# Jiraiya812/Fast-CU-Decision-HEVC

Hardware: AMD Instinct MI355X
Metric: CTUs/sec (RDO decision only) at 4K all-intra (higher is better)
Workload: dtype int32+f64

## Files before the change

### fast-cu-decision-hevc_amd/csrc/fcu_engine.h

```cpp
#pragma once
#include <stdint.h>
#include <string.h>
#include <type_traits>
#include "../../include/fcu.h"

#ifdef FCU_EMU
#include <math.h>
#include <stdio.h>
#include <stdlib.h>
#define FCU_DEV static inline
#define FCU_MEMBER inline
#define FCU_NOINLINE
#define FCU_INLINE
#define FCU_TABLE static const
static int g_emu_phase = 0, g_emu_in_phase = 0, g_emu_lane = 0, g_emu_relax = 0;
#define FCU_EMU_RELAX(on) (g_emu_relax = (on))
static inline int fcu_emu_phase_begin() { g_emu_phase++; g_emu_in_phase = 1; g_emu_lane = 0; return 0; }
static inline int fcu_emu_phase_next(int lane) { if (lane + 1 >= 64) g_emu_in_phase = 0; g_emu_lane = lane + 1; return lane + 1; }
template <class T> static inline T fcu_emu_uni(T v, int site, int line)
{
  enum { SITES = 2048, K = 32, B = 16 };
  struct Seen { int phase, first, cur, idx, n; unsigned char vals[K][B]; };
  static Seen seen[SITES];
  if (g_emu_in_phase && !g_emu_relax && sizeof(T) <= B && site < SITES) {
// ... 927 lines not shown
        rdCodedLevelandDist += cc - cs;
        rdUncodedDist += c0;
        if (posInCG != 0) nnzBeforePos0++;
      }
    }
    if (lastScanPos >= 0 && cgScanPos > 0) {
      ctxSet = (uint32_t)((ch ? 4 : 0) + ((!ch && (cgScanPos - 1) > 0) ? 2 : 0) + (c1 == 0));
      c1 = 1; c2 = 0; c1Idx = 0; c2Idx = 0; goRice = 0;
    }
    if (cgLastScanPos >= 0) {
      if (cgScanPos) {
        if (((cgflag >> cgBlk) & 1) == 0) {
          const int ctxSig = cgBase + sig_cg_ctx(cgflag, cgx, cgy, wg);
          baseCost += lambda * (double)cb(ctxSig, 0) - rdSigCost;
          cgg[cgScanPos * st] = lambda * (double)cb(ctxSig, 0);
        } else if (cgScanPos < cgLastScanPos) {
          if (nnzBeforePos0 == 0) { baseCost -= rdSigCost0; rdSigCost -= rdSigCost0; }
          double costZeroCG = baseCost;
          const int ctxSig = cgBase + sig_cg_ctx(cgflag, cgx, cgy, wg);
          baseCost += lambda * (double)cb(ctxSig, 1);
          costZeroCG += lambda * (double)cb(ctxSig, 0);
          cgg[cgScanPos * st] = lambda * (double)cb(ctxSig, 1);
          costZeroCG += rdUncodedDist; costZeroCG -= rdCodedLevelandDist; costZeroCG -= rdSigCost;
          if (costZeroCG < baseCost) {
            cgflag &= ~(1ull << cgBlk); baseCost = costZeroCG;
            cgg[cgScanPos * st] = lambda * (double)cb(ctxSig, 0);
            for (int posInCG = 15; posInCG >= 0; posInCG--) {
              const int scanPos = cgScanPos * 16 + posInCG;
              if (SER) { if (g_S.rq_lv[posInCG]) { g_S.rq_lv[posInCG] = 0; g_S.rq_rec[posInCG].cc = g_S.rq_rec[posInCG].c0; g_S.rq_rec[posInCG].cs = 0; } }
              else if (dstg[scanPos * st]) { dstg[scanPos * st] = 0; recg[scanPos * st].cc = recg[scanPos * st].c0; recg[scanPos * st].cs = 0; }
            }
          }
        }
      } else cgflag |= 1ull << cgBlk;
    }
    if (SER) {
#pragma unroll
      for (int k = 0; k < 16; k++) { recg[(cgScanPos * 16 + k) * st] = g_S.rq_rec[k]; dstg[(cgScanPos * 16 + k) * st] = g_S.rq_lv[k]; }
    }
  }
  FCU_RTOC(P, rt_, 12);
  if (lastScanPos < 0) { RdoqOut z = { 0, -1 }; return z; }
  return rdoq_finish<SER>(cb, P, srcg, dstg, recg, cgg, st, log2, ch, scanType, cbfCtx, scan, scanCG, cgflag, cgLastScanPos, lastScanPos, baseCost, blockUncodedCost, lambda);
}

#ifdef FCU_EMU
template <class T> struct LaneVar {
  T v[64];
  LaneVar() { for (int i = 0; i < 64; i++) v[i] = T(); }
  void set(int lane, T x) { v[lane] = x; }
  T own(int lane) const { return v[lane]; }
  T get(int k) const { return v[k]; }
  void put(int k, T x) { v[k] = x; }
};
FCU_DEV uint32_t lane_mask16(const LaneVar<int> &f) { uint32_t m = 0; for (int k = 0; k < 16; k++) m |= (uint32_t)(f.v[k] != 0) << k; return m; }
#else
#if defined(__HIP_DEVICE_COMPILE__)
#define FCU_READLANE(v, k) __builtin_amdgcn_readlane((v), (k))
#define FCU_WRITELANE(val_, k_, old_) (((int)threadIdx.x == (k_)) ? (val_) : (old_))
#define FCU_BALLOT(p) __builtin_amdgcn_ballot_w64(p)
#else
#define FCU_READLANE(v, k) (v)
#define FCU_WRITELANE(val_, k_, old_) (val_)
#define FCU_BALLOT(p) ((unsigned long long)(p))
#endif
template <class T> struct LaneVar;
template <> struct LaneVar<int> {
  int r = 0;
  __device__ void set(int, int x) { r = x; }
  __device__ int own(int) const { return r; }
  __device__ int get(int k) const { return FCU_READLANE(r, k); }
  __device__ void put(int k, int x) { r = FCU_WRITELANE(x, k, r); }
};
template <> struct LaneVar<double> {
  double r = 0;
  __device__ void set(int, double x) { r = x; }
  __device__ double own(int) const { return r; }
  __device__ double get(int k) const
  { union { double d; int i[2]; } u; u.d = r; u.i[0] = FCU_READLANE(u.i[0], k); u.i[1] = FCU_READLANE(u.i[1], k); return u.d; }
  __device__ void put(int k, double x)
  { union { double d; int i[2]; } u, w; u.d = r; w.d = x; u.i[0] = FCU_WRITELANE(w.i[0], k, u.i[0]); u.i[1] = FCU_WRITELANE(w.i[1], k, u.i[1]); r = u.d; }
};
__device__ inline uint32_t lane_mask16(const LaneVar<int> &f) { return (uint32_t)FCU_BALLOT(f.r != 0) & 0xffffu; }
#endif

#ifndef FCU_WAVE_RDOQ_MIN_LOG2
#define FCU_WAVE_RDOQ_MIN_LOG2 2
#endif
FCU_DEV FCU_NOINLINE void rdoq_wave(int c, const int32_t *src, int16_t *dst, int topNZ, int log2, int comp, int scanType, int cbfCtx, const Params &P_, RdoqRec *rec, double *costCGSig)
{
  const Params &P = *FCU_UNI(&P_);
  c = FCU_UNI(c); src = FCU_UNI(src); dst = FCU_UNI(dst); topNZ = FCU_UNI(topNZ); log2 = FCU_UNI(log2); comp = FCU_UNI(comp);
  scanType = FCU_UNI(scanType); cbfCtx = FCU_UNI(cbfCtx); rec = FCU_UNI(rec); costCGSig = FCU_UNI(costCGSig);
  if (topNZ < 0) { FCU_SERIAL { g_S.rw_abs = 0; g_S.rw_lsp = -1; } return; }
  const FCU_HBM int32_t *srcg = (const FCU_HBM int32_t *)src; FCU_HBM int16_t *dstg = (FCU_HBM int16_t *)dst;
  FCU_HBM RdoqRec *recg = (FCU_HBM RdoqRec *)rec; FCU_HBM double *cgg = (FCU_HBM double *)costCGSig;
  auto cb = [&](int ctx, int bin) -> int { return (int)FCU_EST[ctx * 2 + bin]; };
  const int ch = comp ? 1 : 0, N = 1 << log2, n2 = N * N;
  const int qp = comp ? P.qp_c : P.qp;
  const int qbits = rdoq_qbits(log2, qp);
  const double lambda = P.rdoq_lambda[comp];
  const double errScale = P.err_scale[ch][log2 - 2];
  const uint16_t *scan = log2 == 2 ? &g_hot.scan[scanType][0] : k_scan + k_scan_off[scanType * 4 + log2 - 2];
  const uint8_t *scanCG = log2 <= 3 ? g_hot.scan_cg8[log2 == 2 ? 0 : scanType] : k_scan_cg + k_scan_cg_off[scanType * 4 + log2 - 2];
  const int wg = N >> 2, firstSig = first_sig_ctx(log2, scanType, ch);
  const int sigOff = CTX_SIG + (ch ? 28 : 0), cgBase = CTX_SIGCG + (ch ? 2 : 0);
  const uint64_t scan4 = g_hot.scan4_nib[scanType], map4 = g_hot.map4_nib;
  const int cgTop = topNZ >> 4;
  uint64_t cgflag = 0;
  int cgLastScanPos = -1; uint32_t ctxSet = 0; int c1 = 1, c2 = 0;
  double baseCost = 0, blockUncodedCost = 0;
  int lastScanPos = -1; uint32_t c1Idx = 0, c2Idx = 0, goRice = 0;
  int g10 = 0, g10Ctx = -1;
  for (int cg = (n2 >> 4) - 1; cg > cgTop; cg -= 4) {
    LaneVar<double> t0;
    FCU_FOR_LANES { const int g = cg - (lane >> 4); if (g > cgTop) { const double err = (double)iabs(srcg[g * 16 + (lane & 15)]); t0.set(lane, err * err * errScale); } }
    for (int j = 0; j < 4 && cg - j > cgTop; j++)
      for (int k = 15; k >= 0; k--) blockUncodedCost += t0.get(j * 16 + k);
  }
  baseCost = blockUncodedCost;
  LaneVar<int> vCgBlk, vNext;
  LaneVar<double> vCgSig;
  FCU_FOR_LANES { if (lane <= cgTop) vCgBlk.set(lane, scanCG[lane]); if (lane < 16) vNext.set(lane, srcg[cgTop * 16 + lane]); }
  for (int cgScanPos = cgTop; cgScanPos >= 0; cgScanPos--) {
    const int cgBlk = vCgBlk.get(cgScanPos), cgy = cgBlk / wg, cgx = cgBlk - cgy * wg;
    const int sigBase = sigOff + firstSig + ((!ch && (cgx + cgy) > 0) ? 3 : 0);
    const uint32_t cntBits = g_hot.cnt_bits[pattern_sig_ctx(cgflag, cgx, cgy, wg)];
    LaneVar<int> vLd, vMax, vSb0, vSb1, vUp, vDn, vSd, vDu, vLv, vCand;
    LaneVar<double> vC0, vCs, vCc;
    FCU_FOR_LANES {
      if (lane < 16) {
        const int posInCG = lane, scanPos = cgScanPos * 16 + posInCG;
        const int32_t levelDouble = iabs(vNext.own(lane));
        if (cgScanPos > 0) vNext.set(lane, srcg[scanPos - 16]);
        uint32_t maxAbsLevel = (uint32_t)((levelDouble + ((int32_t)1 << (qbits - 1))) >> qbits);
        if (maxAbsLevel > 32767u) maxAbsLevel = 32767u;
// ... 139 lines not shown
        if (lane <= top) {
          const int scanPos = cgScanPos * 16 + lane;
          const int lv = dstg[scanPos];
          const RdoqRec q = recg[scanPos];
          wLv.set(lane, lv); wCs.set(lane, q.cs); wCc.set(lane, q.cc); wC0.set(lane, q.c0);
          double costLast = 0;
          if (lv) {
            const int blk = scan[scanPos];
            const int py = blk >> log2, px = blk - (py << log2);
            const int ax = scanType == 2 ? py : px, ay = scanType == 2 ? px : py;
            const int gx = g_hot.group_idx[ax], gy = g_hot.group_idx[ay];
            int bxs = 0, bys = 0;
            for (int k = 0; k < gx; k++) bxs += cb(lbx + (k >> lsh), 1);
            if (gx < lgmax) bxs += cb(lbx + (gx >> lsh), 0);
            for (int k = 0; k < gy; k++) bys += cb(lby + (k >> lsh), 1);
            if (gy < lgmax) bys += cb(lby + (gy >> lsh), 0);
            double r = (double)(bxs + bys);
            if (gx > 3) r += 32768.0 * (double)((gx - 2) >> 1);
            if (gy > 3) r += 32768.0 * (double)((gy - 2) >> 1);
            costLast = lambda * r;
          }
          wCl.set(lane, costLast);
        }
      }
      for (int posInCG = top; posInCG >= 0; posInCG--) {
        const int lv = wLv.get(posInCG); const double curCs = wCs.get(posInCG);
        if (lv) {
          const double totalCost = baseCost + wCl.get(posInCG) - curCs;
          if (totalCost < bestCost) { bestLastIdxP1 = cgScanPos * 16 + posInCG + 1; bestCost = totalCost; }
          if (lv > 1) { foundLast = 1; break; }
          baseCost -= wCc.get(posInCG); baseCost += wC0.get(posInCG);
        } else baseCost -= curCs;
      }
    }
  }
  FCU_SERIAL { g_S.rw_abs = 0; }
  FCU_FOR_LANES {
    uint32_t acc = 0;
    for (int sp = lane; sp <= lastScanPos; sp += 64) {
      if (sp < bestLastIdxP1) { const int lv = dstg[sp]; acc += (uint32_t)lv; dstg[sp] = (int16_t)((srcg[sp] < 0) ? -lv : lv); }
      else dstg[sp] = 0;
    }
    FCU_WAVE_ADD((uint32_t *)&g_S.rw_abs, acc);
  }
  FCU_SERIAL {
    const int absSum = g_S.rw_abs;
    rdoq_sign_hiding(P, srcg, dstg, recg, 1, ch, bestLastIdxP1, absSum);
    int last = bestLastIdxP1 - 1;
    while (last >= 0 && dstg[last] == 0) last--;
    g_S.rw_lsp = last;
  }
}

FCU_DEV int use_filtered_ref(int mode, int log2, int isLuma)
{
  if (!isLuma || mode == DC) return 0;
  const int d1 = iabs(mode - HOR), d2 = iabs(mode - VER);
  return (d1 < d2 ? d1 : d2) > k_filter_thr[log2 - 2];
}
FCU_DEV int pred_pixel(const uint8_t *ref, int log2, int mode, int isLuma, int dc, int x, int y)
{
  const int N = 1 << log2;
  const uint8_t *corner = ref + 2 * N;
  if (mode == PLANAR)
    return ((N - 1 - x) * corner[-1 - y] + (x + 1) * corner[1 + N] + (N - 1 - y) * corner[1 + x] + (y + 1) * corner[-1 - N] + N) >> (log2 + 1);
  if (mode == DC) {
    int v = dc;
    if (isLuma && N <= 16) {
      if (x == 0 && y == 0) v = (corner[1] + corner[-1] + 2 * dc + 2) >> 2;
      else if (y == 0) v = (corner[1 + x] + 3 * dc + 2) >> 2;
      else if (x == 0) v = (corner[-1 - y] + 3 * dc + 2) >> 2;
    }
    return v;
  }
  const int isVer = mode >= 18;
  const int angMode = isVer ? mode - VER : -(mode - HOR);
  const int absAng = iabs(angMode);
  const int angAbs = (int)((0x2069544d245080ull >> (6 * absAng)) & 63);
  const int invAngle = absAng == 0 ? 0 : (int)(((absAng <= 4 ? 0x13b0e38ccd000ull : 0x8004ec30c1e2ull) >> (13 * ((absAng - 1) & 3))) & 8191);
  const int angle = angMode < 0 ? -angAbs : angAbs;
  const int px = isVer ? x : y, py = isVer ? y : x, ms = isVer ? 1 : -1;
  if (angle == 0) {
    int v = corner[ms * (px + 1)];
    if (isLuma && N <= 16 && px == 0) v = clip8(v + ((corner[-ms * (py + 1)] - corner[0]) >> 1));
    return v;
  }
  const int deltaPos = (py + 1) * angle, di = deltaPos >> 5, df = deltaPos & 31;
  const int i0 = px + di + 1;
  int r0, r1;
  { int i = i0; r0 = (i >= 0) ? corner[ms * i] : corner[-ms * ((128 + (-i) * invAngle) >> 8)]; }
  if (!df) return r0;
  { int i = i0 + 1; r1 = (i >= 0) ? corner[ms * i] : corner[-ms * ((128 + (-i) * invAngle) >> 8)]; }
  return ((32 - df) * r0 + df * r1 + 16) >> 5;
}

FCU_DEV int unit_available(const Env E, int lx, int ly, int cx, int cy)
{
  const Params &P = E.C->p;
  if (lx < 0 || ly < 0 || lx >= P.width || ly >= P.height) return 0;
  const int ctuN = (ly >> 6) * E.C->w_ctu + (lx >> 6), ctuC = (cy >> 6) * E.C->w_ctu + (cx >> 6);
  if (ctuN < E.slice_start) return 0;
  if (ctuN < ctuC) return 1;
  if (ctuN > ctuC) return 0;
  return zidx_of(lx, ly) < zidx_of(cx, cy);
}

// ... 778 lines not shown
      while (shift < numFull && cost < candCost[numFull - 1 - shift]) shift++;
      if (shift != 0) {
        for (int i = 1; i < shift; i++) { g_S.rd_mode[numFull - i] = g_S.rd_mode[numFull - 1 - i]; candCost[numFull - i] = candCost[numFull - 1 - i]; }
        g_S.rd_mode[numFull - shift] = mode; candCost[numFull - shift] = cost;
      }
    }
    for (int j = 0; j < nm; j++) {
      int inc = 0;
      for (int i = 0; i < numFull; i++) inc |= (preds[j] == g_S.rd_mode[i]);
      if (!inc) g_S.rd_mode[numFull++] = preds[j];
    }
    g_S.n_rd = numFull;
  }
}

FCU_DEV FCU_NOINLINE void pu_first_pass_batched(CuObj *cu, uint32_t tu_k)
{
  const Env E = env_get(); cu = FCU_UNI(cu); const TU tu = tu_of_key(FCU_UNI(tu_k));
  Scratch *G = E.G; const Params &P = E.C->p;
  const int d = cu->depth_cu, N = 1 << tu.log2, log2 = tu.log2, n2 = N * N, part = tu.part;
  const int partSize = cu->part_size[part];
  int checkTS = P.transform_skip && log2 == 2;
  if (P.ts_fast) checkTS = checkTS && (partSize == SIZE_NxN);
  const int nc = g_S.n_rd, tsv = checkTS ? 2 : 1, tss = tsv - 1, nvc = nc * tsv;
  FCU_CHECK(nvc <= MAXVC && nvc * n2 <= POOL && (MAXLC % 2) == 0);
  const int qbits = rdoq_qbits(log2, P.qp), qscale = k_quant_scales[P.qp % 6];
  const int useDst = log2 == 2;
  const uint8_t *org = G->org[d].y + tu.y * 64 + tu.x;
  build_ref(0, cu->x + tu.x, cu->y + tu.y, log2, 1);
  FCU_FOR_LANES {
    const int dc = g_S.dc;
    for (int i = lane; i < nc * n2; i += 64) {
      const int cnd = i / n2, p = i - cnd * n2, y = p >> log2, x = p & (N - 1), mode = g_S.rd_mode[cnd];
      const uint8_t *r = use_filtered_ref(mode, log2, 1) ? g_S.reff : g_S.ref;
      const int v = pred_pixel(r, log2, mode, 1, dc, x, y);
      G->p_pred[i] = (uint8_t)v; G->p_resi[i] = (int16_t)(org[y * 64 + x] - v);
    }
  }
  FCU_FOR_LANES { if (lane < nvc) g_S.vc_last[lane] = -1; by_log2(log2, [&](auto L) { constexpr int LG = decltype(L)::value; RowCache<(1 << LG), int16_t> rc; for (int i = lane; i < nc * n2; i += 64) { const int cnd = i / n2; G->p_tmp[i] = fwd1<LG>(rc, G->p_resi + cnd * n2, useDst, i - cnd * n2); } }); }
  FCU_FOR_LANES {
    est_build(CAB_CUR0 + d, lane);
    by_log2(log2, [&](auto L) { constexpr int LG = decltype(L)::value; RowCache<(1 << LG), int32_t> rc;
      for (int i = lane; i < nvc * n2; i += 64) {
        const int v = i / n2, p = i - v * n2, cnd = (v >> tss), ts = (v & tss);
        const uint16_t *iscan = k_iscan + k_scan_off[coef_scan_idx(g_S.rd_mode[cnd], log2, 0) * 4 + log2 - 2];
        const int32_t t = ts ? ((int32_t)G->p_resi[cnd * n2 + p] << (15 - 8 - log2)) : fwd2<LG>(rc, G->p_tmp + cnd * n2, useDst, p);
        const int sp = iscan[p]; const int32_t ld = level_double(t, qscale, qbits);
        G->p_lscan[sp * nvc + v] = ld;
        if (level_nonzero(ld, qbits)) FCU_ATOMIC_MAX(&g_S.vc_last[v], sp);
      }
    });
  }
  FCU_TIC(t2_);
  FCU_FOR_LANES {
    if (lane < nvc) {
      const int mode = g_S.rd_mode[(lane >> tss)];
      RdoqRec *rrec = G->r_rec + lane; double *rcg = G->r_cg + lane;
      const int cbfCtx = CTX_CBF_LUMA + (tu.tr_depth == 0 ? 1 : 0);
      const RdoqOut o = ((lane & tss) ? P.rdoq_ts : P.rdoq) ? rdoq<0, 1>(CAB_CUR0 + d, G->p_lscan + lane, G->p_qscan + lane, nvc, g_S.vc_last[lane], log2, 0, coef_scan_idx(mode, log2, 0), cbfCtx, P, rrec, rcg)
                                                            : quant_plain(G->p_lscan + lane, G->p_qscan + lane, nvc, g_S.vc_last[lane], log2, 0, P);
      g_S.vc_abs[lane] = o.abs_sum; g_S.vc_lsp[lane] = o.last;
      g_S.vc_dist[lane] = 0;
    }
    if (lane == 0) E.C->n_tu_trials += (unsigned long long)nvc;
  }
  FCU_TOC(E, t2_, 2);
  FCU_FOR_LANES {
    const DeqParams dq = deq_params(log2, P.qp);
    for (int i = lane; i < nvc * n2; i += 64) {
      const int v = i / n2, p = i - v * n2;
      const uint16_t *iscan = k_iscan + k_scan_off[coef_scan_idx(g_S.rd_mode[(v >> tss)], log2, 0) * 4 + log2 - 2];
      const int sp = iscan[p];
      const int q = (g_S.vc_abs[v] > 0 && (sp >> 4) <= (g_S.vc_last[v] >> 4)) ? G->p_qscan[sp * nvc + v] : 0;
      G->p_tmp[((v & tss)) ? i : v * n2 + tr_index(p, log2)] = dequant1(q, dq);
    }
  }
  FCU_FOR_LANES {
    by_log2(log2, [&](auto L) { constexpr int LG = decltype(L)::value; RowCache<(1 << LG), int32_t> rc;
      for (int i = lane; i < nvc * n2; i += 64) {
        const int v = i / n2, p = i - v * n2, ts = (v & tss);
        if (ts) { const int s = 15 - 8 - log2; G->p_tcoef[i] = (G->p_tmp[i] + (1 << (s - 1))) >> s; }
        else G->p_tcoef[i] = inv1<LG>(rc, G->p_tmp + v * n2, useDst, p);
      }
    });
  }
  FCU_FOR_LANES {
    by_log2(log2, [&](auto L) {
      uint32_t acc = 0;
      for (int i = lane; i < nvc * n2; i += 64) {
        const int v = i / n2, p = i - v * n2, cnd = (v >> tss), ts = (v & tss), y = p >> log2, x = p & (N - 1);
        int res = 0;
        if (g_S.vc_abs[v] > 0) res = ts ? (int16_t)G->p_tcoef[i] : inv2<decltype(L)::value>(G->p_tcoef + v * n2, useDst, p);
        const int r = clip8(G->p_pred[cnd * n2 + p] + res);
        G->p_rec[i] = (uint8_t)r;
        const int e = org[y * 64 + x] - r;
        FCU_DIST_ADD(acc, v, e, i, n2);
      }
    });
  }
  FCU_TIC(t3_);
  for (int vbase = 0; vbase < nvc; vbase += MAXLC) {
    const int slotBase = vbase ? (g_S.vc_slot[g_S.pu_best_vc] + 1) % MAXLC : 0;
#if defined(FCU_EMU) && defined(FCU_EMU_TRACE_ROUNDS)
    if (vbase) fprintf(stderr, "second bit-count round: %d variants\n", nvc);
#endif
    FCU_FOR_LANES {
      const int vc = vbase + lane;
      if (lane < MAXLC && vc < nvc) {
        const int cnd = (vc >> tss), ts = (vc & tss), mode = g_S.rd_mode[cnd], cbf = g_S.vc_abs[vc] > 0;
        const int slot = (slotBase + lane) % MAXLC;
        double cost;
        g_S.vc_slot[vc] = (uint8_t)slot;
        if (ts && !cbf) cost = FCU_MAX_DOUBLE;
        else {
          const int c = CAB_LANE0 + slot;
          cab_copy1(&g_S.cab[c], slot_ptr(E, d, CI_CURR_BEST));
          cab_reset_bits(c);
          if (part == 0 && P.slice_type != SLICE_I) { code_skip_flag(E, c, cu, 0); code_pred_mode(c, cu, 0); }
// ... 31 lines not shown
      }
      for (int i = lane; i < tu.nparts; i += 64) { G->tmp_tr_idx[i] = (uint8_t)tu.tr_depth; G->tmp_cbf[i] = (uint8_t)(cbf << tu.tr_depth); G->tmp_tskip[i] = (uint8_t)ts; }
    }
  }
}

FCU_DEV FCU_NOINLINE void pu_first_pass_64(CuObj *cu, uint32_t root_k)
{
  const Env E = env_get(); cu = FCU_UNI(cu); const TU root = tu_of_key(FCU_UNI(root_k));
  Scratch *G = E.G; const Params &P = E.C->p;
  const int d = cu->depth_cu, nc = g_S.n_rd, log2 = 5, N = 32, n2 = N * N, partSize = cu->part_size[root.part];
  FCU_CHECK(nc <= 5 && nc * n2 <= POOL && root.log2 == 6);
  const int qbits = rdoq_qbits(log2, P.qp), qscale = k_quant_scales[P.qp % 6];
  uint8_t *recpic = E.C->rec[0] + cu->y * E.C->stride[0] + cu->x; const int rs = E.C->stride[0];
  FCU_FOR_LANES {
    if (lane < nc) { const int c = CAB_LANE0 + lane; cab_copy1(&g_S.cab[c], slot_ptr(E, d, CI_CURR_BEST)); cab_reset_bits(c); g_S.c64_dist[lane] = 0; }
  }
  for (int k = 0; k < 4; k++) {
    TU tu; tu_child(tu, root, k, 0);
    const uint8_t *org = G->org[d].y + tu.y * 64 + tu.x;
    for (int cand = 0; cand < nc; cand++) {
      const int mode = g_S.rd_mode[cand], filt = use_filtered_ref(mode, log2, 1);
      if (k) {
        FCU_FOR_LANES {
          for (int i = lane; i < k * n2; i += 64) {
            const int j = i >> 10, q = i & (n2 - 1), yy = (j >> 1) * N + (q >> log2), xx = (j & 1) * N + (q & (N - 1));
            recpic[yy * rs + xx] = G->c64_rec[cand][yy * 64 + xx];
          }
        }
      }
      build_ref(0, cu->x + tu.x, cu->y + tu.y, log2, filt);
      FCU_FOR_LANES {
        const uint8_t *r = filt ? g_S.reff : g_S.ref; const int dc = g_S.dc;
        for (int i = lane; i < n2; i += 64) {
          const int y = i >> log2, x = i & (N - 1);
          const int v = pred_pixel(r, log2, mode, 1, dc, x, y);
          G->p_pred[cand * n2 + i] = (uint8_t)v; G->p_resi[cand * n2 + i] = (int16_t)(org[y * 64 + x] - v);
        }
      }
    }
    FCU_FOR_LANES { if (lane < nc) g_S.vc_last[lane] = -1; by_log2(log2, [&](auto L) { constexpr int LG = decltype(L)::value; RowCache<(1 << LG), int16_t> rc; for (int i = lane; i < nc * n2; i += 64) { const int cnd = i / n2; G->p_tmp[i] = fwd1<LG>(rc, G->p_resi + cnd * n2, 0, i - cnd * n2); } }); }
    FCU_FOR_LANES {
      by_log2(log2, [&](auto L) { constexpr int LG = decltype(L)::value; RowCache<(1 << LG), int32_t> rc;
        for (int i = lane; i < nc * n2; i += 64) {
          const int v = i / n2, p = i - v * n2;
          const uint16_t *iscan = k_iscan + k_scan_off[coef_scan_idx(g_S.rd_mode[v], log2, 0) * 4 + log2 - 2];
          const int32_t t = fwd2<LG>(rc, G->p_tmp + v * n2, 0, p);
          const int sp = iscan[p]; const int32_t ld = level_double(t, qscale, qbits);
          G->p_lscan[sp * nc + v] = ld;
          if (level_nonzero(ld, qbits)) FCU_ATOMIC_MAX(&g_S.vc_last[v], sp);
        }
      });
    }
    FCU_FOR_LANES {
      if (lane < nc) {
        RdoqRec *rrec = G->r_rec + lane; double *rcg = G->r_cg + lane;
        const RdoqOut o = P.rdoq ? rdoq<0, 0>(CAB_LANE0 + lane, G->p_lscan + lane, G->p_qscan + lane, nc, g_S.vc_last[lane], log2, 0,
                                              coef_scan_idx(g_S.rd_mode[lane], log2, 0), CTX_CBF_LUMA + (tu.tr_depth == 0 ? 1 : 0), P, rrec, rcg)
                                 : quant_plain(G->p_lscan + lane, G->p_qscan + lane, nc, g_S.vc_last[lane], log2, 0, P);
        g_S.vc_abs[lane] = o.abs_sum; g_S.vc_lsp[lane] = o.last; g_S.vc_dist[lane] = 0;
      }
      if (lane == 0) E.C->n_tu_trials += (unsigned long long)nc;
    }
    FCU_FOR_LANES {
      const DeqParams dq = deq_params(log2, P.qp);
      for (int i = lane; i < nc * n2; i += 64) {
        const int v = i / n2, p = i - v * n2;
        const uint16_t *iscan = k_iscan + k_scan_off[coef_scan_idx(g_S.rd_mode[v], log2, 0) * 4 + log2 - 2];
        const int sp = iscan[p];
        const int q = (g_S.vc_abs[v] > 0 && (sp >> 4) <= (g_S.vc_last[v] >> 4)) ? G->p_qscan[sp * nc + v] : 0;
        G->c64_coef[v][tu.off_y + sp] = (int16_t)q;
        G->p_tmp[v * n2 + tr_index(p, log2)] = dequant1(q, dq);
      }
    }
    FCU_FOR_LANES { by_log2(log2, [&](auto L) { constexpr int LG = decltype(L)::value; RowCache<(1 << LG), int32_t> rc; for (int i = lane; i < nc * n2; i += 64) { const int v = i / n2; G->p_tcoef[i] = inv1<LG>(rc, G->p_tmp + v * n2, 0, i - v * n2); } }); }
    FCU_FOR_LANES {
      by_log2(log2, [&](auto L) {
        uint32_t acc = 0;
        for (int i = lane; i < nc * n2; i += 64) {
          const int v = i / n2, p = i - v * n2, y = p >> log2, x = p & (N - 1);
          const int res = g_S.vc_abs[v] > 0 ? inv2<decltype(L)::value>(G->p_tcoef + v * n2, 0, p) : 0;
          const int r = clip8(G->p_pred[i] + res);
          G->c64_rec[v][(tu.y + y) * 64 + tu.x + x] = (uint8_t)r;
          const int e = org[y * 64 + x] - r;
          FCU_DIST_ADD(acc, v, e, i, n2);
        }
      });
    }
    FCU_FOR_LANES {
      if (lane < nc) {
        const int c = CAB_LANE0 + lane, mode = g_S.rd_mode[lane], cbf = g_S.vc_abs[lane] > 0;
        if (tu.part == 0 && P.slice_type != SLICE_I) { code_skip_flag(E, c, cu, 0); code_pred_mode(c, cu, 0); }
        if (tu.part == 0 && d == MAXDEPTH) cab_bin(c, partSize == SIZE_2Nx2N, CTX_PARTSIZE);
        if (tu.part == 0) code_luma_dir_bits(c, mode, g_S.preds);
        if (log2 != LOG2_MINTU && log2 != min_tu_log2_in_cu(d, partSize)) cab_bin(c, 0, CTX_SUBDIV + 5 - log2);
        cab_bin(c, cbf, CTX_CBF_LUMA + (tu.tr_depth == 0 ? 1 : 0));
        if (cbf) code_coeff_nxn<0>(c, G->p_qscan + lane, nc, g_S.vc_lsp[lane], log2, 0, coef_scan_idx(mode, log2, 0), 0, P, g_S.lane_abs[lane]);
        g_S.c64_dist[lane] += g_S.vc_dist[lane]; g_S.c64_cbf[lane][k] = (uint8_t)cbf;
        G->c64_distk[lane][k] = g_S.vc_dist[lane]; cab_copy1(&G->c64_state[lane][k], &g_S.cab[c]);
      }
    }
  }
  FCU_SERIAL {
    double best = FCU_MAX_DOUBLE; int bv = 0;
    for (int cand = 0; cand < nc; cand++) {
      const double c = rd_cost(P, (uint32_t)(g_S.cab[CAB_LANE0 + cand].frac >> 15), g_S.c64_dist[cand]);
      if (c < best) { best = c; bv = cand; }
    }
    g_S.pu_best_vc = bv; g_S.pu_best_cost = best; g_S.pu_best_dist = g_S.c64_dist[bv]; g_S.pu_best_mode = g_S.rd_mode[bv];
    g_S.c64_valid = 1;
  }
  {
    const int bv = g_S.pu_best_vc;
    Yuv *reco = &G->reco[d][1 - g_S.reco_best_idx[d]];
    const int any = g_S.c64_cbf[bv][0] | g_S.c64_cbf[bv][1] | g_S.c64_cbf[bv][2] | g_S.c64_cbf[bv][3];
    FCU_FOR_LANES {
// ... 152 lines not shown
    }
  }
  FCU_EMU_RELAX(0);
  return cab_bits(c);
}

FCU_DEV FCU_NOINLINE void chroma_leaf_trials(CuObj *cu, uint32_t tu_k)
{
  const Env E = env_get(); cu = FCU_UNI(cu); const TU tu = tu_of_key(FCU_UNI(tu_k));
  Scratch *G = E.G; const Params &P = E.C->p;
  const int d = cu->depth_cu;
  const int N = tu.cw, log2 = ilog2(N), n2 = N * N, trDepth = tu.tr_depth;
  int checkTS = P.transform_skip && N <= 4;
  if (P.ts_fast) {
    checkTS = checkTS && (tu.log2 == 2);
    if (checkTS) { int nb = 0; const int maxp = tu.part + (tu.c_code_all ? 1 : 4); for (int p = tu.part; p < maxp; p++) nb += cu->tskip[0][p]; checkTS = checkTS && (nb > 0); }
  }
  const int tsv = checkTS ? 2 : 1, tss = tsv - 1;
  const int perRound = (tsv == 1 && 10 * n2 <= POOL) ? 2 : 1;
  const int nm = 5 * perRound, nvc = nm * tsv;
  const int qbits = rdoq_qbits(log2, P.qp_c), qscale = k_quant_scales[P.qp_c % 6];
  const int subPart = tu_part_c(tu), nPartsC = tu_nparts_c(tu);
  const int lumaDir = cu->intra_dir[0][tu.part & ~3];
  for (int comp0 = 1; comp0 < 3; comp0 += perRound) {
    const int px = (cu->x >> 1) + tu.cx, py = (cu->y >> 1) + tu.cy;
    for (int cc = 0; cc < perRound; cc++) {
      const int comp = comp0 + cc;
      const uint8_t *org = yuv_plane(&G->org[d], comp) + tu.cy * 32 + tu.cx;
      chroma_leaf_refs5(E, cu, comp, px, py, log2);
      FCU_FOR_LANES {
        for (int i = lane; i < 5 * n2; i += 64) {
          const int m = i / n2, p = i - m * n2, y = p >> log2, x = p & (N - 1);
          const int mode = g_S.c_modes[m] == DM_CHROMA ? lumaDir : g_S.c_modes[m];
          const int pr = pred_pixel(g_S.ref5[m], log2, mode, 0, g_S.dc5[m], x, y);
          G->p_pred[cc * 5 * n2 + i] = (uint8_t)pr; G->p_resi[cc * 5 * n2 + i] = (int16_t)(org[y * 32 + x] - pr);
        }
      }
    }
    FCU_FOR_LANES { if (lane < nvc) g_S.vc_last[lane] = -1; by_log2(log2, [&](auto L) { constexpr int LG = decltype(L)::value; RowCache<(1 << LG), int16_t> rc; for (int i = lane; i < nm * n2; i += 64) { const int b = i / n2; G->p_tmp[i] = fwd1<LG>(rc, G->p_resi + b * n2, 0, i - b * n2); } }); }
    FCU_FOR_LANES {
      by_log2(log2, [&](auto L) { constexpr int LG = decltype(L)::value; RowCache<(1 << LG), int32_t> rc;
        for (int i = lane; i < nvc * n2; i += 64) {
          const int v = i / n2, p = i - v * n2, b = (v >> tss), ts = (v & tss), m = b % 5, comp = comp0 + b / 5;
          const int mode = g_S.c_modes[m] == DM_CHROMA ? lumaDir : g_S.c_modes[m];
          const uint16_t *iscan = k_iscan + k_scan_off[coef_scan_idx(mode, log2, comp) * 4 + log2 - 2];
          const int32_t t = ts ? ((int32_t)G->p_resi[b * n2 + p] << (15 - 8 - log2)) : fwd2<LG>(rc, G->p_tmp + b * n2, 0, p);
          const int sp = iscan[p]; const int32_t ld = level_double(t, qscale, qbits);
          G->p_lscan[sp * nvc + v] = ld;
          if (level_nonzero(ld, qbits)) FCU_ATOMIC_MAX(&g_S.vc_last[v], sp);
        }
      });
    }
    FCU_TIC(t13_);
    FCU_FOR_LANES {
      if (lane < nvc) {
        const int b = (lane >> tss), m = b % 5, comp = comp0 + b / 5;
        const int mode = g_S.c_modes[m] == DM_CHROMA ? lumaDir : g_S.c_modes[m];
        RdoqRec *rrec = G->r_rec + lane; double *rcg = G->r_cg + lane;
        const RdoqOut o = ((lane & tss) ? P.rdoq_ts : P.rdoq)
          ? rdoq<0, 0>(CAB_LANE0 + m, G->p_lscan + lane, G->p_qscan + lane, nvc, g_S.vc_last[lane], log2, 1 , coef_scan_idx(mode, log2, comp), CTX_CBF_CHROMA + trDepth, P, rrec, rcg)
          : quant_plain(G->p_lscan + lane, G->p_qscan + lane, nvc, g_S.vc_last[lane], log2, 1, P);
        g_S.vc_abs[lane] = o.abs_sum; g_S.vc_lsp[lane] = o.last;
        g_S.vc_dist[lane] = 0;
      }
      if (lane == 0) E.C->n_tu_trials += (unsigned long long)nvc;
    }
    FCU_TOC(E, t13_, 13);
    FCU_FOR_LANES {
      const DeqParams dq = deq_params(log2, P.qp_c);
      for (int i = lane; i < nvc * n2; i += 64) {
        const int v = i / n2, p = i - v * n2, b = (v >> tss), m = b % 5, comp = comp0 + b / 5;
        const int mode = g_S.c_modes[m] == DM_CHROMA ? lumaDir : g_S.c_modes[m];
        const uint16_t *iscan = k_iscan + k_scan_off[coef_scan_idx(mode, log2, comp) * 4 + log2 - 2];
        const int sp = iscan[p];
        const int q = (g_S.vc_abs[v] > 0 && (sp >> 4) <= (g_S.vc_last[v] >> 4)) ? G->p_qscan[sp * nvc + v] : 0;
        G->p_tmp[((v & tss)) ? i : v * n2 + tr_index(p, log2)] = dequant1(q, dq);
      }
    }
    FCU_FOR_LANES {
      by_log2(log2, [&](auto L) { constexpr int LG = decltype(L)::value; RowCache<(1 << LG), int32_t> rc;
        for (int i = lane; i < nvc * n2; i += 64) {
          const int v = i / n2, p = i - v * n2, ts = (v & tss);
          if (ts) { const int sft = 15 - 8 - log2; G->p_tcoef[i] = (G->p_tmp[i] + (1 << (sft - 1))) >> sft; }
          else G->p_tcoef[i] = inv1<LG>(rc, G->p_tmp + v * n2, 0, p);
        }
      });
    }
    FCU_FOR_LANES {
      by_log2(log2, [&](auto L) {
        uint32_t acc = 0;
        for (int i = lane; i < nvc * n2; i += 64) {
          const int v = i / n2, p = i - v * n2, b = (v >> tss), ts = (v & tss), y = p >> log2, x = p & (N - 1);
          const uint8_t *org = yuv_plane(&G->org[d], comp0 + b / 5) + tu.cy * 32 + tu.cx;
          int res = 0;
          if (g_S.vc_abs[v] > 0) res = ts ? (int16_t)G->p_tcoef[i] : inv2<decltype(L)::value>(G->p_tcoef + v * n2, 0, p);
          const int r = clip8(G->p_pred[b * n2 + p] + res);
          G->p_rec[i] = (uint8_t)r;
          const int e = org[y * 32 + x] - r;
          FCU_DIST_ADD(acc, v, e, i, n2);
        }
      });
    }
    FCU_FOR_LANES {
      if (lane < 5) {
        const int m = lane; int bestTs = 0;
        const int mode = g_S.c_modes[m] == DM_CHROMA ? lumaDir : g_S.c_modes[m];
        if (tsv == 2) {
          const int comp = comp0;
          uint32_t dsel = (uint32_t)(P.chroma_weight * (double)g_S.vc_dist[m * 2]);
          const uint32_t d0 = dsel, d1 = (uint32_t)(P.chroma_weight * (double)g_S.vc_dist[m * 2 + 1]);
          const int c0 = CAB_LANE0 + 5 + m, c1 = CAB_LANE0 + 10 + m;
          cab_copy1(&g_S.cab[c0], &g_S.cab[CAB_LANE0 + m]); cab_reset_bits(c0);
          if (g_S.vc_abs[m * 2] > 0) code_coeff_nxn<0>(c0, G->p_qscan + m * 2, nvc, g_S.vc_lsp[m * 2], log2, comp, coef_scan_idx(mode, log2, comp), 0, P, g_S.lane_abs[lane]);
          const double cost0 = rd_cost(P, cab_bits(c0), d0);
          double cost1 = FCU_MAX_DOUBLE;
          if (g_S.vc_abs[m * 2 + 1] > 0) {
            cab_copy1(&g_S.cab[c1], &g_S.cab[CAB_LANE0 + m]); cab_reset_bits(c1);
            code_coeff_nxn<0>(c1, G->p_qscan + m * 2 + 1, nvc, g_S.vc_lsp[m * 2 + 1], log2, comp, coef_scan_idx(mode, log2, comp), 1, P, g_S.lane_abs[lane]);
            cost1 = rd_cost(P, cab_bits(c1), d1);
// ... 517 lines not shown
```

Baseline: 18580.

## Batch RDOQ across candidates with lane-parallel sig-context precompute

Replaces the per-lane serial RDOQ call for each candidate TU with a batched walker. All candidates advance coefficient group by coefficient group in lockstep. Within each group, spare wave lanes precompute level magnitudes and significance bit costs for several scan positions at once. They also write records for zero coefficients directly, and the owning lanes then consume these values through ds_bpermute. The aim is to cut serial per-lane latency and divergence when nvc is much smaller than the wave width, at the cost of more lane shuffles, extra per-lane state and a large new code path.

```diff
diff --git a/fast-cu-decision-hevc_amd/csrc/fcu_engine.h b/fast-cu-decision-hevc_amd/csrc/fcu_engine.h
--- a/fast-cu-decision-hevc_amd/csrc/fcu_engine.h
+++ b/fast-cu-decision-hevc_amd/csrc/fcu_engine.h
@@ -1003,17 +1003,21 @@
   T own(int lane) const { return v[lane]; }
   T get(int k) const { return v[k]; }
   void put(int k, T x) { v[k] = x; }
+  T pull(int k) const { return v[k]; }
 };
 FCU_DEV uint32_t lane_mask16(const LaneVar<int> &f) { uint32_t m = 0; for (int k = 0; k < 16; k++) m |= (uint32_t)(f.v[k] != 0) << k; return m; }
+template <class T> struct LaneOwn { T v[64]; T &at(int lane) { return v[lane]; } };
 #else
 #if defined(__HIP_DEVICE_COMPILE__)
 #define FCU_READLANE(v, k) __builtin_amdgcn_readlane((v), (k))
 #define FCU_WRITELANE(val_, k_, old_) (((int)threadIdx.x == (k_)) ? (val_) : (old_))
 #define FCU_BALLOT(p) __builtin_amdgcn_ballot_w64(p)
+#define FCU_PULL(v, k) __builtin_amdgcn_ds_bpermute((k) << 2, (v))
 #else
 #define FCU_READLANE(v, k) (v)
 #define FCU_WRITELANE(val_, k_, old_) (val_)
 #define FCU_BALLOT(p) ((unsigned long long)(p))
+#define FCU_PULL(v, k) (v)
 #endif
 template <class T> struct LaneVar;
 template <> struct LaneVar<int> {
@@ -1022,6 +1026,7 @@
   __device__ int own(int) const { return r; }
   __device__ int get(int k) const { return FCU_READLANE(r, k); }
   __device__ void put(int k, int x) { r = FCU_WRITELANE(x, k, r); }
+  __device__ int pull(int k) const { return FCU_PULL(r, k); }
 };
 template <> struct LaneVar<double> {
   double r = 0;
@@ -1033,6 +1038,7 @@
   { union { double d; int i[2]; } u, w; u.d = r; w.d = x; u.i[0] = FCU_WRITELANE(w.i[0], k, u.i[0]); u.i[1] = FCU_WRITELANE(w.i[1], k, u.i[1]); r = u.d; }
 };
 __device__ inline uint32_t lane_mask16(const LaneVar<int> &f) { return (uint32_t)FCU_BALLOT(f.r != 0) & 0xffffu; }
+template <class T> struct LaneOwn { T r; __device__ T &at(int) { return r; } };
 #endif
 
 #ifndef FCU_WAVE_RDOQ_MIN_LOG2
@@ -1278,6 +1284,238 @@
   }
 }
 
+FCU_DEV int rdoq_batch_desc(int coder, int scanType, int useRdoq) { return coder | (scanType << 8) | (useRdoq << 10); }
+struct RdoqWalk {
+  uint64_t cgflag;
+  double baseCost, blockUncodedCost, rdSigCost, rdSigCost0, rdCodedLevelandDist, rdUncodedDist;
+  int cgTop, cgBlk, cgLastScanPos, lastScanPos, c1, c2, g10, g10Ctx, nnzBeforePos0, nzMask;
+  uint32_t ctxSet, c1Idx, c2Idx, goRice;
+};
+template <int EST>
+FCU_DEV FCU_NOINLINE void rdoq_batch(LaneVar<int> vDesc, int nvc, int log2, int comp, int cbfCtx, const Params &P_, const int32_t *src, int16_t *dst, RdoqRec *rec, double *costCGSig)
+{
+  const Params &P = *FCU_UNI(&P_);
+  nvc = FCU_UNI(nvc); log2 = FCU_UNI(log2); comp = FCU_UNI(comp); cbfCtx = FCU_UNI(cbfCtx);
+  src = FCU_UNI(src); dst = FCU_UNI(dst); rec = FCU_UNI(rec); costCGSig = FCU_UNI(costCGSig);
+  const FCU_HBM int32_t *srcg = (const FCU_HBM int32_t *)src; FCU_HBM int16_t *dstg = (FCU_HBM int16_t *)dst;
+  FCU_HBM RdoqRec *recg = (FCU_HBM RdoqRec *)rec; FCU_HBM double *cgg = (FCU_HBM double *)costCGSig;
+  auto cbv = [&](int coder, int ctx, int bin) -> int { return EST ? (int)FCU_EST[ctx * 2 + bin] : ctx_bits(coder, ctx, bin); };
+  const int st = nvc, ch = comp ? 1 : 0, N = 1 << log2, n2 = N * N;
+  const int qp = comp ? P.qp_c : P.qp, qbits = rdoq_qbits(log2, qp);
+  const double lambda = P.rdoq_lambda[comp], errScale = P.err_scale[ch][log2 - 2];
+  const int wg = N >> 2, sigOff = CTX_SIG + (ch ? 28 : 0), cgBase = CTX_SIGCG + (ch ? 2 : 0);
+  const uint64_t map4 = g_hot.map4_nib;
+  const int lpad = nvc <= 4 ? 2 : (nvc <= 8 ? 3 : (nvc <= 16 ? 4 : 5)), pad = 1 << lpad, ppr = 64 >> lpad, rounds = 16 / ppr;
+  LaneOwn<RdoqWalk> wk;
+  LaneVar<int> vTop, vGrp, vCnt;
+
+  auto begin_group = [&](RdoqWalk &W, int lane, int cg) {
+    const int desc = vDesc.own(lane), scanType = (desc >> 8) & 3;
+    int g = 0; uint32_t cnt = 0;
+    if (cg >= 0 && cg <= W.cgTop) {
+      const uint8_t *scanCG = log2 <= 3 ? g_hot.scan_cg8[log2 == 2 ? 0 : scanType] : k_scan_cg + k_scan_cg_off[scanType * 4 + log2 - 2];
+      const int cgBlk = scanCG[cg], cgy = cgBlk / wg, cgx = cgBlk - cgy * wg;
+      const int sigBase = sigOff + first_sig_ctx(log2, scanType, ch) + ((!ch && (cgx + cgy) > 0) ? 3 : 0);
+      cnt = g_hot.cnt_bits[pattern_sig_ctx(W.cgflag, cgx, cgy, wg)];
+      W.cgBlk = cgBlk;
+      W.rdSigCost = 0; W.rdSigCost0 = 0; W.rdCodedLevelandDist = 0; W.rdUncodedDist = 0; W.nnzBeforePos0 = 0; W.nzMask = 0;
+      cgg[cg * st + lane] = 0;
+      g = 1 | (scanType << 1) | (sigBase << 3) | ((desc & 255) << 11);
+    }
+    vGrp.set(lane, g); vCnt.set(lane, (int)cnt);
+  };
+  auto walk_step = [&](RdoqWalk &W, int lane, int cg, int posInCG, int32_t levelDouble, int sbit0, int sbit1) {
+    const int scanPos = cg * 16 + posInCG, coder = vDesc.own(lane) & 255;
+    uint32_t maxAbsLevel = (uint32_t)((levelDouble + ((int32_t)1 << (qbits - 1))) >> qbits);
+    if (maxAbsLevel > 32767u) maxAbsLevel = 32767u;
+    const double err = (double)levelDouble;
+    double c0 = err * err * errScale, cc = 0, cs = 0;
+    W.blockUncodedCost += c0;
+    uint32_t level = maxAbsLevel;
+    if (maxAbsLevel > 0 && W.lastScanPos < 0) {
+      W.lastScanPos = scanPos;
+      W.ctxSet = (uint32_t)((ch ? 4 : 0) + ((!ch && (scanPos >> 4) > 0) ? 2 : 0));
+      W.cgLastScanPos = cg;
+    }
+    if (W.lastScanPos >= 0) {
+      const int oneCtx = CTX_ONE + 4 * (int)W.ctxSet + W.c1;
+      if (oneCtx != W.g10Ctx) { W.g10 = cbv(coder, oneCtx, 0); W.g10Ctx = oneCtx; }
+      if (maxAbsLevel == 0) {
+        cs = lambda * (double)sbit0; cc = c0 + cs;
+        recg[scanPos * st + lane].up = W.g10;
+        W.baseCost += cc;
+        W.rdSigCost += cs;
+        if (posInCG == 0) W.rdSigCost0 = cs;
+        return;
+      }
+      auto cbs = [&](int, int bin) -> int { return bin ? sbit1 : sbit0; };
+      int sdel = 0, rup, rdn = 0;
+      const int absCtx = CTX_ABS + (int)W.ctxSet + W.c2;
+      LevelBits lb; lb.g10 = W.g10; lb.g11 = cbv(coder, oneCtx, 1); lb.g20 = cbv(coder, absCtx, 0); lb.g21 = cbv(coder, absCtx, 1);
+      int rateHi = 0, rateLo = 0;
+      if (scanPos == W.lastScanPos)
+        level = coded_level(cbs, lambda, &cc, &c0, &cs, levelDouble, maxAbsLevel, 0, lb, W.goRice, W.c1Idx, W.c2Idx, qbits, errScale, 1, &rateHi, &rateLo);
+      else {
+        level = coded_level(cbs, lambda, &cc, &c0, &cs, levelDouble, maxAbsLevel, 0, lb, W.goRice, W.c1Idx, W.c2Idx, qbits, errScale, 0, &rateHi, &rateLo);
+        sdel = sbit1 - sbit0;
+      }
+      if (level > 0) {
+        if (level == maxAbsLevel) {
+          rup = ic_rate(lb, level + 1, W.goRice, W.c1Idx, W.c2Idx) - rateHi;
+          rdn = (maxAbsLevel > 1 ? rateLo : ic_rate(lb, 0, W.goRice, W.c1Idx, W.c2Idx)) - rateHi;
+        } else {
+          rup = rateHi - rateLo;
+          rdn = ic_rate(lb, level - 1, W.goRice, W.c1Idx, W.c2Idx) - rateLo;
+        }
+      } else rup = lb.g10;
+      RdoqRec q; q.cc = cc; q.cs = cs; q.c0 = c0; q.up = rup; q.dn = rdn; q.sd = sdel;
+      q.du = (int32_t)((levelDouble - ((int32_t)level << qbits)) >> (qbits - 8));
+      recg[scanPos * st + lane] = q;
+      W.baseCost += cc;
+      const uint32_t baseLevel = (W.c1Idx < 8) ? (2 + (W.c2Idx < 1)) : 1;
+      if (level >= baseLevel) { if (level > 3u * (1u << W.goRice)) W.goRice = W.goRice + 1 < 4 ? W.goRice + 1 : 4; }
+      if (level >= 1) W.c1Idx++;
+      if (level > 1) { W.c1 = 0; W.c2 += (W.c2 < 2); W.c2Idx++; }
+      else if (W.c1 < 3 && W.c1 > 0 && level) W.c1++;
+    } else W.baseCost += c0;
+    if (maxAbsLevel > 0) dstg[scanPos * st + lane] = (int16_t)level;
+    W.rdSigCost += cs;
+    if (posInCG == 0) W.rdSigCost0 = cs;
+    if (level) {
+      W.cgflag |= 1ull << W.cgBlk;
+      W.rdCodedLevelandDist += cc - cs;
+      W.rdUncodedDist += c0;
+      if (posInCG != 0) W.nnzBeforePos0++;
+      W.nzMask |= 1 << posInCG;
+    }
+  };
+  auto end_group = [&](RdoqWalk &W, int lane, int cg) {
+    const int coder = vDesc.own(lane) & 255, cgBlk = W.cgBlk, cgy = cgBlk / wg, cgx = cgBlk - cgy * wg;
+    if (W.lastScanPos >= 0 && cg > 0) {
+      W.ctxSet = (uint32_t)((ch ? 4 : 0) + ((!ch && (cg - 1) > 0) ? 2 : 0) + (W.c1 == 0));
+      W.c1 = 1; W.c2 = 0; W.c1Idx = 0; W.c2Idx = 0; W.goRice = 0;
+    }
+    if (W.cgLastScanPos >= 0) {
+      if (cg) {
+        if (((W.cgflag >> cgBlk) & 1) == 0) {
+          const int ctxSig = cgBase + sig_cg_ctx(W.cgflag, cgx, cgy, wg);
+          W.baseCost += lambda * (double)cbv(coder, ctxSig, 0) - W.rdSigCost;
+          cgg[cg * st + lane] = lambda * (double)cbv(coder, ctxSig, 0);
+        } else if (cg < W.cgLastScanPos) {
+          if (W.nnzBeforePos0 == 0) { W.baseCost -= W.rdSigCost0; W.rdSigCost -= W.rdSigCost0; }
+          double costZeroCG = W.baseCost;
+          const int ctxSig = cgBase + sig_cg_ctx(W.cgflag, cgx, cgy, wg);
+          W.baseCost += lambda * (double)cbv(coder, ctxSig, 1);
+          costZeroCG += lambda * (double)cbv(coder, ctxSig, 0);
+          cgg[cg * st + lane] = lambda * (double)cbv(coder, ctxSig, 1);
+          costZeroCG += W.rdUncodedDist; costZeroCG -= W.rdCodedLevelandDist; costZeroCG -= W.rdSigCost;
+          if (costZeroCG < W.baseCost) {
+            W.cgflag &= ~(1ull << cgBlk); W.baseCost = costZeroCG;
+            cgg[cg * st + lane] = lambda * (double)cbv(coder, ctxSig, 0);
+            for (uint32_t m = (uint32_t)W.nzMask; m; m &= m - 1) {
+              const int i = (cg * 16 + __builtin_ctz(m)) * st + lane;
+              dstg[i] = 0; recg[i].cc = recg[i].c0; recg[i].cs = 0;
+            }
+          }
+        }
+      } else W.cgflag |= 1ull << cgBlk;
+    }
+  };
+
+  FCU_FOR_LANES {
+    if (lane < nvc) {
+      RdoqWalk &W = wk.at(lane);
+      const int desc = vDesc.own(lane), topNZ = g_S.vc_last[lane];
+      W.cgTop = (((desc >> 10) & 1) && topNZ >= 0) ? topNZ >> 4 : -1;
+      W.cgflag = 0; W.cgLastScanPos = -1; W.lastScanPos = -1; W.ctxSet = 0; W.c1 = 1; W.c2 = 0;
+      W.c1Idx = 0; W.c2Idx = 0; W.goRice = 0; W.g10 = 0; W.g10Ctx = -1; W.blockUncodedCost = 0;
+      if (W.cgTop >= 0) {
+        for (int cg = (n2 >> 4) - 1; cg > W.cgTop; cg--) {
+          int32_t v[16];
+#pragma unroll
+          for (int k = 0; k < 16; k++) v[k] = srcg[(cg * 16 + k) * st + lane];
+#pragma unroll
+          for (int k = 15; k >= 0; k--) { const double err = (double)iabs(v[k]); W.blockUncodedCost += err * err * errScale; }
+        }
+      }
+      W.baseCost = W.blockUncodedCost;
+      vTop.set(lane, W.cgTop);
+    }
+  }
+  int cgMax = -1;
+  for (int v = 0; v < nvc; v++) { const int t = vTop.get(v); cgMax = t > cgMax ? t : cgMax; }
+  if (cgMax >= 0) FCU_FOR_LANES { if (lane < nvc) begin_group(wk.at(lane), lane, cgMax); }
+  for (int cg = cgMax; cg >= 0; cg--) {
+    for (int r = 0; r < rounds; r++) {
+      LaneVar<int> vLd, vS0, vS1;
+      FCU_FOR_LANES {
+        const int v = lane & (pad - 1), k = lane >> lpad;
+        const int g = vGrp.pull(v), cnt = vCnt.pull(v);
+        if (v < nvc && (g & 1)) {
+          const int posInCG = 15 - (r * ppr + k), scanPos = cg * 16 + posInCG, scanType = (g >> 1) & 3, coder = g >> 11;
+          const int32_t levelDouble = iabs(srcg[scanPos * st + v]);
+          uint32_t maxAbsLevel = (uint32_t)((levelDouble + ((int32_t)1 << (qbits - 1))) >> qbits);
+          if (maxAbsLevel > 32767u) maxAbsLevel = 32767u;
+          const int p4 = (int)((g_hot.scan4_nib[scanType] >> (4 * posInCG)) & 15);
+          int ctxSig;
+          if (log2 == 2) ctxSig = sigOff + (p4 ? (int)((map4 >> (4 * p4)) & 15) : 0);
+          else if (scanPos == 0) ctxSig = sigOff;
+          else ctxSig = ((g >> 3) & 255) + (int)(((uint32_t)cnt >> (2 * p4)) & 3);
+          const int sbit0 = cbv(coder, ctxSig, 0), sbit1 = cbv(coder, ctxSig, 1);
+          vLd.set(lane, levelDouble); vS0.set(lane, sbit0); vS1.set(lane, sbit1);
+          if (maxAbsLevel == 0) {
+            const double err = (double)levelDouble;
+            const double c0 = err * err * errScale, cs = lambda * (double)sbit0;
+            RdoqRec q; q.cc = c0 + cs; q.cs = cs; q.c0 = c0; q.up = 0; q.dn = 0; q.sd = sbit1 - sbit0; q.du = (int32_t)(levelDouble >> (qbits - 8));
+            recg[scanPos * st + v] = q;
+            dstg[scanPos * st + v] = 0;
+          }
+        }
+      }
+      FCU_FOR_LANES {
+        const int v = lane & (pad - 1);
+        int ld = vLd.pull(v), s0 = vS0.pull(v), s1 = vS1.pull(v);
+        for (int k = 0; k < ppr; k++) {
+          const int kn = ((k + 1 < ppr ? k + 1 : k) << lpad) | v;
+          const int nld = vLd.pull(kn), ns0 = vS0.pull(kn), ns1 = vS1.pull(kn);
+          if (lane < nvc) { RdoqWalk &W = wk.at(lane); if (cg <= W.cgTop) walk_step(W, lane, cg, 15 - (r * ppr + k), ld, s0, s1); }
+          ld = nld; s0 = ns0; s1 = ns1;
+        }
+        if (r == rounds - 1 && lane < nvc) {
+          RdoqWalk &W = wk.at(lane);
+          if (cg <= W.cgTop) end_group(W, lane, cg);
+          begin_group(W, lane, cg - 1);
+        }
+      }
+    }
+  }
+  FCU_FOR_LANES {
+    const int desc = vDesc.own(lane);
+    if (lane < nvc && ((desc >> 10) & 1)) {
+      RdoqWalk &W = wk.at(lane);
+      const int coder = desc & 255, scanType = (desc >> 8) & 3;
+      RdoqOut o = { 0, -1 };
+      if (W.lastScanPos >= 0) {
+        auto cb = [&](int ctx, int bin) -> int { return cbv(coder, ctx, bin); };
+        const uint16_t *scan = log2 == 2 ? &g_hot.scan[scanType][0] : k_scan + k_scan_off[scanType * 4 + log2 - 2];
+        const uint8_t *scanCG = log2 <= 3 ? g_hot.scan_cg8[log2 == 2 ? 0 : scanType] : k_scan_cg + k_scan_cg_off[scanType * 4 + log2 - 2];
+        o = rdoq_finish<0>(cb, P, srcg + lane, dstg + lane, recg + lane, cgg + lane, st, log2, ch, scanType, cbfCtx, scan, scanCG,
+                           W.cgflag, W.cgLastScanPos, W.lastScanPos, W.baseCost, W.blockUncodedCost, lambda);
+      }
+      g_S.vc_abs[lane] = o.abs_sum; g_S.vc_lsp[lane] = o.last;
+    }
+  }
+}
+FCU_DEV void quant_plain_batch(const LaneVar<int> &vDesc, int nvc, int log2, int comp, const Params &P, const int32_t *src, int16_t *dst)
+{
+  FCU_FOR_LANES {
+    if (lane < nvc && !((vDesc.own(lane) >> 10) & 1)) {
+      const RdoqOut o = quant_plain(src + lane, dst + lane, nvc, g_S.vc_last[lane], log2, comp, P);
+      g_S.vc_abs[lane] = o.abs_sum; g_S.vc_lsp[lane] = o.last;
+    }
+  }
+}
+
 FCU_DEV int use_filtered_ref(int mode, int log2, int isLuma)
 {
   if (!isLuma || mode == DC) return 0;
@@ -2162,18 +2400,13 @@
     });
   }
   FCU_TIC(t2_);
+  LaneVar<int> vDesc;
   FCU_FOR_LANES {
-    if (lane < nvc) {
-      const int mode = g_S.rd_mode[(lane >> tss)];
-      RdoqRec *rrec = G->r_rec + lane; double *rcg = G->r_cg + lane;
-      const int cbfCtx = CTX_CBF_LUMA + (tu.tr_depth == 0 ? 1 : 0);
-      const RdoqOut o = ((lane & tss) ? P.rdoq_ts : P.rdoq) ? rdoq<0, 1>(CAB_CUR0 + d, G->p_lscan + lane, G->p_qscan + lane, nvc, g_S.vc_last[lane], log2, 0, coef_scan_idx(mode, log2, 0), cbfCtx, P, rrec, rcg)
-                                                            : quant_plain(G->p_lscan + lane, G->p_qscan + lane, nvc, g_S.vc_last[lane], log2, 0, P);
-      g_S.vc_abs[lane] = o.abs_sum; g_S.vc_lsp[lane] = o.last;
-      g_S.vc_dist[lane] = 0;
-    }
+    if (lane < nvc) { vDesc.set(lane, rdoq_batch_desc(CAB_CUR0 + d, coef_scan_idx(g_S.rd_mode[(lane >> tss)], log2, 0), (lane & tss) ? P.rdoq_ts : P.rdoq)); g_S.vc_dist[lane] = 0; }
     if (lane == 0) E.C->n_tu_trials += (unsigned long long)nvc;
   }
+  rdoq_batch<1>(vDesc, nvc, log2, 0, CTX_CBF_LUMA + (tu.tr_depth == 0 ? 1 : 0), P, G->p_lscan, G->p_qscan, G->r_rec, G->r_cg);
+  if (!P.rdoq || (tss && !P.rdoq_ts)) quant_plain_batch(vDesc, nvc, log2, 0, P, G->p_lscan, G->p_qscan);
   FCU_TOC(E, t2_, 2);
   FCU_FOR_LANES {
     const DeqParams dq = deq_params(log2, P.qp);
@@ -2311,16 +2544,13 @@
         }
       });
     }
+    LaneVar<int> vDesc;
     FCU_FOR_LANES {
-      if (lane < nc) {
-        RdoqRec *rrec = G->r_rec + lane; double *rcg = G->r_cg + lane;
-        const RdoqOut o = P.rdoq ? rdoq<0, 0>(CAB_LANE0 + lane, G->p_lscan + lane, G->p_qscan + lane, nc, g_S.vc_last[lane], log2, 0,
-                                              coef_scan_idx(g_S.rd_mode[lane], log2, 0), CTX_CBF_LUMA + (tu.tr_depth == 0 ? 1 : 0), P, rrec, rcg)
-                                 : quant_plain(G->p_lscan + lane, G->p_qscan + lane, nc, g_S.vc_last[lane], log2, 0, P);
-        g_S.vc_abs[lane] = o.abs_sum; g_S.vc_lsp[lane] = o.last; g_S.vc_dist[lane] = 0;
-      }
+      if (lane < nc) { vDesc.set(lane, rdoq_batch_desc(CAB_LANE0 + lane, coef_scan_idx(g_S.rd_mode[lane], log2, 0), P.rdoq)); g_S.vc_dist[lane] = 0; }
       if (lane == 0) E.C->n_tu_trials += (unsigned long long)nc;
     }
+    rdoq_batch<0>(vDesc, nc, log2, 0, CTX_CBF_LUMA + (tu.tr_depth == 0 ? 1 : 0), P, G->p_lscan, G->p_qscan, G->r_rec, G->r_cg);
+    if (!P.rdoq) quant_plain_batch(vDesc, nc, log2, 0, P, G->p_lscan, G->p_qscan);
     FCU_FOR_LANES {
       const DeqParams dq = deq_params(log2, P.qp);
       for (int i = lane; i < nc * n2; i += 64) {
@@ -2579,19 +2809,18 @@
       });
     }
     FCU_TIC(t13_);
+    LaneVar<int> vDesc;
     FCU_FOR_LANES {
       if (lane < nvc) {
         const int b = (lane >> tss), m = b % 5, comp = comp0 + b / 5;
         const int mode = g_S.c_modes[m] == DM_CHROMA ? lumaDir : g_S.c_modes[m];
-        RdoqRec *rrec = G->r_rec + lane; double *rcg = G->r_cg + lane;
-        const RdoqOut o = ((lane & tss) ? P.rdoq_ts : P.rdoq)
-          ? rdoq<0, 0>(CAB_LANE0 + m, G->p_lscan + lane, G->p_qscan + lane, nvc, g_S.vc_last[lane], log2, 1 , coef_scan_idx(mode, log2, comp), CTX_CBF_CHROMA + trDepth, P, rrec, rcg)
-          : quant_plain(G->p_lscan + lane, G->p_qscan + lane, nvc, g_S.vc_last[lane], log2, 1, P);
-        g_S.vc_abs[lane] = o.abs_sum; g_S.vc_lsp[lane] = o.last;
+        vDesc.set(lane, rdoq_batch_desc(CAB_LANE0 + m, coef_scan_idx(mode, log2, comp), (lane & tss) ? P.rdoq_ts : P.rdoq));
         g_S.vc_dist[lane] = 0;
       }
       if (lane == 0) E.C->n_tu_trials += (unsigned long long)nvc;
     }
+    rdoq_batch<0>(vDesc, nvc, log2, 1, CTX_CBF_CHROMA + trDepth, P, G->p_lscan, G->p_qscan, G->r_rec, G->r_cg);
+    if (!P.rdoq || (tss && !P.rdoq_ts)) quant_plain_batch(vDesc, nvc, log2, 1, P, G->p_lscan, G->p_qscan);
     FCU_TOC(E, t13_, 13);
     FCU_FOR_LANES {
       const DeqParams dq = deq_params(log2, P.qp_c);
```

Result: faster. 18820 (median of 6 runs) (+1.3%).
